# tachyon-beep/keisei

Hardware: AMD Instinct MI355X
Metric: PPO samples/sec, se_resnet 40x256 on 50x9x9 (higher is better)
Workload: dtype bf16; 1 GPU; se_resnet 40x256 KataGo-PPO minibatch step (gather+fwd+loss+bwd+clip+Adam), minibatch 4096/GPU from a 16384-sample device-resident epoch dataset, obs 50x9x9; per_gpu_batch=4096, global_batch=4096, parallelism=dp1

## Files before the change

include/keisei_amd.h:

```cpp
#ifndef KEISEI_AMD_H
#define KEISEI_AMD_H

#ifdef __cplusplus
extern "C" {
#endif

#define KA_OK 0
#define KA_ERR_ARG (-1)
#define KA_ERR_HIP (-2)
#define KA_ERR_UNSUPPORTED (-3)
#define KA_DTYPE_F32 0
#define KA_DTYPE_BF16 1

int ka_version(void);
const char* ka_target_arch(void);
const char* ka_last_error(void);
int ka_options_reload(void);

int ka_conv3x3_fwd(const void* in, const void* wpack, void* out, const float* in_scale, const float* in_shift,
                   const float* in_bias, int relu, float* bsum, float* sqpart, int B, int Cin, int Cout, int dtype,
                   void* stream);
int ka_conv3x3_fwd_keep_supported(int B, int Cin, int Cout, int dtype);
int ka_conv3x3_fwd_keep(const void* in, const void* wpack, void* out, const float* in_scale, const float* in_shift,
                        const float* in_bias, int relu, float* bsum, float* sqpart, void* x_out, int B, int Cin, int Cout, int dtype,
                        void* stream);
int ka_conv3x3_sqpart_rows(int B);
int ka_conv_route_counts(long long* out, int n);
int ka_conv3x3_dgrad_fused(const void* in, const void* in2, const float* k, void* dy_out, const void* wpack, void* out,
                           float* bsum, const void* ep_y, const float* ep_scale, const float* ep_shift,
                           const float* ep_mean, const float* ep_invstd, float* ep_s1, float* ep_s2, int B, int Cin,
                           int Cout, int dtype, void* stream);
int ka_conv3x3_dgrad_gated_supported(int B, int Cin, int Cout, int dtype, int masked);
int ka_conv3x3_dgrad_fused_gated(const void* du, const float* gate_add, const void* in2, const float* k,
                                 void* dy_out, const void* wpack, void* out, float* bsum, const void* ep_y,
                                 const float* ep_scale, const float* ep_shift, const float* ep_mean, const float* ep_invstd,
                                 float* ep_s1, float* ep_s2, int B, int Cin, int Cout, int dtype, void* stream);
int ka_pack_conv3x3(const float* w, void* dst, int Co, int Ci, int Nout, int Kin, int mode, int dtype, void* stream);
int ka_pack_conv3x3_multi(const long long* table, int n, long long max_pieces, int dtype, void* stream);
int ka_conv3x3_wgrad(const void* dy, const void* x, const float* in_scale, const float* in_shift, const float* in_bias,
                     int relu, float* slab, float* dw, int B, int Cin, int Cin_real, int Cout, int accumulate,
                     int target_wgs, int dtype, void* stream);
int ka_wgrad_splits(int B, int Cin, int Cout, int target_wgs);
int ka_debug_conv_stamps(unsigned long long* stamps);

int ka_obs_to_nhwc(const float* obs, const long long* idx, void* out, int B, int Cobs, int Cpad, int dtype, void* stream);
int ka_nhwc_to_nchw(const void* in, float* out, int B, int C, int dtype, void* stream);

int ka_reduce_workspace_doubles(int C);
int ka_bn_reduce(const float* bsum, int B, const float* sqpart, int R, int C, double* sums, double* part, void* stream);
int ka_bn_coeffs(const double* sums, double count, const double* count_dev, const float* gamma, const float* beta,
                 float* running_mean, float* running_var, long long* num_batches_tracked, float momentum, float eps,
                 float* scale, float* shift, float* mean, float* invstd, int C, void* stream);
int ka_bn_eval_coeffs(const float* gamma, const float* beta, const float* running_mean, const float* running_var,
                      float eps, float* scale, float* shift, int C, void* stream);
int ka_bn_eval_coeffs_multi(const long long* table, int n, int max_c, void* stream);
int ka_pair_reduce(const float* p1, const float* p2, int B, int C, double* sums, double* part, void* stream);
int ka_bn_bwd_coeffs(const double* sums_local, const double* sums_global, double count, const double* count_dev,
                     const float* gamma, const float* mean, const float* invstd, float* dgamma, float* dbeta, float* k,
                     int C, int train, void* stream);
int ka_sync_reduce(const float* p1, int rows1, const float* p2, int rows2, int C, double count, double* sums,
                   double* local_copy, double* part, void* stream);
int ka_bn_coeffs_parts(const double* part, double count, const float* gamma, const float* beta, float* running_mean,
                       float* running_var, long long* num_batches_tracked, float momentum, float eps, float* scale,
                       float* shift, float* mean, float* invstd, int C, void* stream);
int ka_bn_bwd_coeffs_parts(const double* part, double count, const float* gamma, const float* mean, const float* invstd,
                           float* dgamma, float* dbeta, float* k, int C, int train, void* stream);
int ka_bn_reduce_coeffs(const float* bsum, int B, const float* sqpart, int R, int C, double* part, int* counters, double count,
                        const float* gamma, const float* beta, float* running_mean, float* running_var,
                        long long* num_batches_tracked, float momentum, float eps, float* scale, float* shift, float* mean,
                        float* invstd, void* stream);
int ka_pair_reduce_bwd_coeffs(const float* p1, const float* p2, int rows, int C, double* part, int* counters, double count,
                              const float* gamma, const float* mean, const float* invstd, float* dgamma, float* dbeta, float* k,
                              int train, void* stream);
int ka_bn_bwd_apply(const void* dz, const void* y, const float* k, void* dy, int B, int C, int dtype, void* stream);
int ka_affine_rows(const float* in, const float* a, const float* s, float mul, float* out, int B, int C, void* stream);
// ... 287 lines not shown
```

keisei_amd/_lib.py:

```python
from __future__ import annotations

import ctypes
import os
from pathlib import Path
from typing import Optional

import torch

_LIB_PATH = Path(os.environ.get("KEISEI_AMD_LIB") or Path(__file__).resolve().parent / "libkeisei_amd.so")

_SIGS = {
    "ka_conv3x3_fwd": "pppppp i pp iii i p",
    "ka_conv3x3_fwd_keep_supported": "iiii",
    "ka_conv3x3_fwd_keep": "pppppp i pp p iii i p",
    "ka_conv3x3_dgrad_fused": "ppppp pp ppppp pp iii i p",
    "ka_conv3x3_dgrad_gated_supported": "iiiii",
    "ka_conv3x3_dgrad_fused_gated": "pppppp pp ppppp pp iii i p",
    "ka_conv3x3_sqpart_rows": "i",
    "ka_conv_route_counts": "p i",
    "ka_debug_conv_stamps": "p",
    "ka_pack_conv3x3": "pp iiii i i p",
    "ka_pack_conv3x3_multi": "p i q i p",
    "ka_wgrad_splits": "iiii",
    "ka_conv3x3_wgrad": "ppppp i pp iiii i i i p",
    "ka_obs_to_nhwc": "ppp iii i p",
    "ka_nhwc_to_nchw": "pp ii i p",
    "ka_bn_reduce": "p i p i i pp p",
    "ka_reduce_workspace_doubles": "i",
    "ka_pair_reduce": "pp ii pp p",
    "ka_sync_reduce": "p i p i i d ppp p",
    "ka_bn_coeffs": "p d p pppp p ff pppp i p",
    "ka_bn_coeffs_parts": "p d pppp p ff pppp i p",
    "ka_bn_bwd_coeffs_parts": "p d ppp ppp i i p",
    "ka_bn_reduce_coeffs": "p i p i i pp d pppp p ff pppp p",
    "ka_pair_reduce_bwd_coeffs": "pp i i pp d ppp ppp i p",
    "ka_bn_eval_coeffs": "pppp f pp i p",
    "ka_bn_bwd_coeffs": "pp d p ppp ppp i i p",
    "ka_affine_rows": "ppp f p ii p",
    "ka_bn_bwd_apply": "pppp ii i p",
    "ka_block_tail_fwd": "ppppp pp ii i p",
    "ka_block_tail_fwd_se_supported": "iii",
    "ka_block_tail_fwd_se": "pppppppp ppp ppp iii i p",
    "ka_pool_fwd": "pp ii i p",
    "ka_tail_bwd_reduce": "pppppp p ii i p",
    "ka_tail_bwd_dz": "ppppppp ppp ii i p",
    "ka_tail_bwd_fused_supported": "iii",
    "ka_tail_bwd_fused": "ppppp pppppp p pppp iii i p",
    "ka_relu_bn_bwd_reduce": "pppppp ppp ii i p",
    "ka_block_dx": "pppppp p ii i p",
    "ka_block_dx_tail_bwd_supported": "iii",
    "ka_block_dx_tail_bwd": "pppppp p ppppppppp p pppp iii i p",
    "ka_block_dx_tail_bwd_du": "ppppp p ppppppppp p pppp iii i p",
    "ka_block_dx_tail_bwd_du_gate": "ppppp p ppppppppp pp pppp iii i p",
    "ka_gemm": "pppp iii iii ii iii i i i p",
    "ka_reduce_slabs": "pp i q i p",
    "ka_reduce_slabs2": "pp q pp q i p",
    "ka_colsum": "pppp ii i p",
# ... 267 lines not shown
```

keisei_amd/csrc/wgrad.hip:

```cpp
#include <stdlib.h>
#include <type_traits>
#include "common.h"

namespace {

constexpr int kTC = 64;

struct WgradArgs {
    const void* dy;
    const void* x;
    const float* in_scale;
    const float* in_shift;
    const float* in_bias;
    float* slab;
    int B, Cin, Cout, relu, boards_per_split, ntn, ntiles, nsplit;
    int stagger;
    unsigned long long* stamps;
};

typedef __attribute__((address_space(3))) bf16x4* lds_bf16x4_ptr;

template <typename T, int TN> struct WG;
template <int TN> struct WG<bf16_t, TN> {
    static constexpr int KROWS = TN == 128 ? 82 : 96;
    static constexpr int PW = TN == 128 ? 17 : 11;
    static constexpr int SY = TN * 2 + 32;
    static constexpr int SX = kTC * 2 + 32;
};
template <int TN> struct WG<float, TN> {
    static constexpr int PW = 11;
    static constexpr int KROWS = 84;
    static constexpr int SY = TN * 4 + 64;
    static constexpr int SX = kTC * 4 + 64;
};

template <typename T, int TN, bool FUSED>
__global__ __launch_bounds__(TN * 4, TN == 64 ? 2 : 1) void wgrad_kernel(WgradArgs a) {
    typedef Elem<T> E;
    typedef typename E::vec16 vec16;
    constexpr int NTHR = TN * 4;
    constexpr int ESZ = E::kSize, P16 = E::kPer16;
    constexpr int SY = WG<T, TN>::SY, SX = WG<T, TN>::SX, KROWS = WG<T, TN>::KROWS;
    constexpr int PW = WG<T, TN>::PW, XSQ = 11 * PW;
    auto xsq = [](int p) { return (p / 9 + 1) * PW + (p % 9) + 1; };
    constexpr int PY = TN * ESZ / 16, PX = kTC * ESZ / 16;
    constexpr int NY = (KA_BOARD * PY + NTHR - 1) / NTHR, NX = (KA_BOARD * PX + NTHR - 1) / NTHR;
    extern __shared__ __attribute__((aligned(16))) char smem[];
    constexpr bool FLAT = sizeof(T) == 2 && TN == 128;
    constexpr int NBUF = FLAT ? 3 : ((sizeof(T) == 2) ? 2 : 1);
    constexpr int TILE_BYTES = KROWS * SY + XSQ * SX;
// ... 206 lines not shown
            }
        }
        }
        if (NBUF >= 2) {
            if (late) stage_next(b, ys, xs);
            __syncthreads();
        }
    };
    if (NSETS == 2) {
        for (int b = bbeg; b < bend; b += 2) {
            board_iter(b, ry[NSETS - 1], rx[NSETS - 1]);
            if (b + 1 < bend) board_iter(b + 1, ry[0], rx[0]);
        }
    } else {
#pragma unroll 1
        for (int b = bbeg; b < bend; ++b) board_iter(b, ry[0], rx[0]);
    }

    if (c_ok) {
        const int c = c0 + cq * 16 + r;
#pragma unroll
        for (int tap = 0; tap < 9; ++tap)
#pragma unroll
            for (int t = 0; t < 4; ++t)
#pragma unroll
                for (int i = 0; i < 4; ++i) {
                    const int n = n0 + (nh * 4 + t) * 16 + q * 4 + i;
                    if (n < a.Cout && c < a.Cin)
                        a.slab[(((size_t)split * 9 + tap) * a.Cout + n) * a.Cin + c] = acc[tap][t][i];
                }
    }
}

template <bool FUSED>
__global__ __launch_bounds__(512, 1) void wgrad_flat_kernel(WgradArgs a) {
    constexpr int NTHR = 512, SY = 128 * 2 + 32, SX = kTC * 2 + 32, KROWS = 82, PW = 17, XSQ = 11 * PW;
    constexpr int YB = KROWS * SY, TILE = YB + XSQ * SX, XTAB = 3 * TILE;
    constexpr int kTapBias = (PW + 1) * SX;
    constexpr bool PIPE = false;
    extern __shared__ __attribute__((aligned(16))) char smem[];
    const int tid = threadIdx.x, lane = tid & 63, wave = __builtin_amdgcn_readfirstlane(tid >> 6);
    const int r = lane & 15, q = lane >> 4;
    const int nh = wave & 1, cq = wave >> 1;
    const int xcd = blockIdx.x & 7, slot = blockIdx.x >> 3;
    const int tile = slot % a.ntiles;
    const int split = xcd + 8 * (slot / a.ntiles);
    if (split >= a.nsplit) return;
    const int tn = tile % a.ntn, tc = tile / a.ntn;
    const int n0 = tn * 128, c0 = tc * kTC;
    const int bbeg = split * a.boards_per_split;
    const int bend = min(a.B, bbeg + a.boards_per_split), nb = bend - bbeg;

    f32x4 acc[9][4];
#pragma unroll
    for (int t = 0; t < 9; ++t)
#pragma unroll
        for (int j = 0; j < 4; ++j) acc[t][j] = f32x4{0.f, 0.f, 0.f, 0.f};
    for (int i = tid; i < 3 * TILE / 16; i += NTHR) reinterpret_cast<uint4*>(smem)[i] = uint4{0, 0, 0, 0};
    if (tid < KROWS) {
        const int p = tid < KA_BOARD ? tid : 0;
        reinterpret_cast<int*>(smem + XTAB)[tid] = YB + ((p / 9 + 1) * PW + (p % 9) + 1) * SX;
    }

    const int yj = tid & 15, xj = tid & 7;
    const bool ycol_ok = n0 + yj * 8 < a.Cout, xcol_ok = c0 + xj * 8 < a.Cin;
    const __amdgpu_buffer_rsrc_t rs_y = __builtin_amdgcn_make_buffer_rsrc(const_cast<void*>(a.dy), 0, (unsigned)a.B * (KA_BOARD * 2u) * (unsigned)a.Cout, 0x00020000);
    const __amdgpu_buffer_rsrc_t rs_x = __builtin_amdgcn_make_buffer_rsrc(const_cast<void*>(a.x), 0, (unsigned)a.B * (KA_BOARD * 2u) * (unsigned)a.Cin, 0x00020000);
    const __amdgpu_buffer_rsrc_t rs_b = __builtin_amdgcn_make_buffer_rsrc(const_cast<float*>(FUSED ? a.in_bias : nullptr), 0,
                                                                          FUSED && a.in_bias ? (unsigned)a.B * 4u * (unsigned)a.Cin : 0u, 0x00020000);
    constexpr int kPark = 0x7fffffff;
    int ldsY[3], gY[3], ldsX[2], gX[2];
#pragma unroll
    for (int i = 0; i < 3; ++i) {
        const int row = (tid >> 4) + 32 * i;
        gY[i] = row < KA_BOARD && ycol_ok ? (row * a.Cout + n0 + yj * 8) * 2 : kPark;
        ldsY[i] = row < KA_BOARD ? row * SY + yj * 16 : 256;
    }
#pragma unroll
    for (int i = 0; i < 2; ++i) {
        const int row = (tid >> 3) + 64 * i;
        gX[i] = row < KA_BOARD && xcol_ok ? (row * a.Cin + c0 + xj * 8) * 2 : kPark;
        ldsX[i] = row < KA_BOARD ? YB + ((row / 9 + 1) * PW + (row % 9) + 1) * SX + xj * 16 : YB + (PW + 1) * SX + kTC * 2;
    }
    const int gB = xcol_ok ? (c0 + xj * 8) * 4 : kPark;
// ... 73 lines not shown
                tf = pad ? s_toff : tf;
            }
            yo[h] = tf + p * SY + coly;
            xo[h] = tf + *reinterpret_cast<const int*>(smem + XTAB + p * 4) + colx - kTapBias;
        }
        s_k += 32; s_p += 32;
        if (s_p >= KA_BOARD) { s_p -= KA_BOARD; s_toff = toff_next; }
    };

    if (a.stamps && tid == 0) {
        a.stamps[blockIdx.x * 8 + 0] = __builtin_amdgcn_s_memtime();
        a.stamps[blockIdx.x * 8 + 3] = __builtin_amdgcn_s_memrealtime();
    }
    if (nb > 0) load_board(bbeg);
    KA_LDS_BARRIER();
    if (nb > 0) {
        store_board(0);
        if (nb > 1) load_board(bbeg + 1);
    }
    prepare();
    KA_LDS_BARRIER();
    int ks = 0;
#ifdef KA_DIAG_WGRAD_TL
#define KA_TL(ph) do { if (a.stamps && blockIdx.x == 0 && jl >= 8 && jl < 24 && lane == 0) \
        a.stamps[4096 * 8 + ((jl - 8) * 8 + wave) * 8 + (ph)] = __builtin_amdgcn_s_memtime(); } while (0)
#else
#define KA_TL(ph) do {} while (0)
#endif
#pragma unroll 1
    for (int jl = 0; jl < nb; ++jl) {
        KA_TL(0);
        const int nxt = ((jl + 1) % 3) * TILE;
        auto stage_next = [&]() {
            if (jl + 1 < nb) {
                store_board(nxt);
                if (jl + 2 < nb) load_board(bbeg + jl + 2);
            }
        };
        if (!late) stage_next();
        KA_TL(1);
        const int ks_hi = jl + 1 == nb ? (KA_BOARD * nb + 31) / 32 : (KA_BOARD * (jl + 1)) / 32;
        if (!skip) {
            auto load_a = [&](bf16x8 (&f)[4]) {
#pragma unroll
                for (int t = 0; t < 4; ++t) {
                    bf16x4 lo = __builtin_amdgcn_ds_read_tr16_b64_v4bf16((lds_bf16x4_ptr)(smem + yo[0] + t * 32));
                    bf16x4 hi = __builtin_amdgcn_ds_read_tr16_b64_v4bf16((lds_bf16x4_ptr)(smem + yo[1] + t * 32));
                    f[t] = __builtin_shufflevector(lo, hi, 0, 1, 2, 3, 4, 5, 6, 7);
                }
            };
            auto kstep = [&](bf16x8 (&ac)[4], bf16x8 (&an)[4], bool more) {
                const int x0 = xo[0], x1 = xo[1];
                auto load_b = [&](int tap) {
                    const int toff = ((tap / 3 - 1) * PW + (tap % 3 - 1)) * SX + kTapBias;
                    bf16x4 lo = __builtin_amdgcn_ds_read_tr16_b64_v4bf16((lds_bf16x4_ptr)(smem + x0 + toff));
                    bf16x4 hi = __builtin_amdgcn_ds_read_tr16_b64_v4bf16((lds_bf16x4_ptr)(smem + x1 + toff));
                    return (bf16x8)__builtin_shufflevector(lo, hi, 0, 1, 2, 3, 4, 5, 6, 7);
                };
                bf16x8 bcur = load_b(0), bnx = load_b(1);
                prepare();
                if (PIPE && more) load_a(an);
#pragma unroll
                for (int tap = 0; tap < 9; ++tap) {
                    bf16x8 bn2 = bnx;
                    if (tap < 7) bn2 = load_b(tap + 2);
#pragma unroll
                    for (int t = 0; t < 4; ++t)
                        acc[tap][t] = __builtin_amdgcn_mfma_f32_16x16x32_bf16(ac[t], bcur, acc[tap][t], 0, 0, 0);
                    bcur = bnx; bnx = bn2;
// ... 26 lines not shown
        KA_TL(4);
    }
#undef KA_TL

    if (a.stamps && tid == 0) {
        a.stamps[blockIdx.x * 8 + 7] = __builtin_amdgcn_s_memtime();
        a.stamps[blockIdx.x * 8 + 4] = __builtin_amdgcn_s_memrealtime();
    }
    if (!skip) {
        const int c = c0 + cq * 16 + r;
        float* sl = a.slab + (size_t)split * 9 * a.Cout * a.Cin;
        const bool whole = n0 + nh * 64 + 64 <= a.Cout && c0 + cq * 16 + 16 <= a.Cin;
        if (whole) {
            float* base = sl + (size_t)(n0 + nh * 64 + q * 4) * a.Cin + c;
#pragma unroll
            for (int tap = 0; tap < 9; ++tap)
#pragma unroll
                for (int t = 0; t < 4; ++t)
#pragma unroll
                    for (int i = 0; i < 4; ++i)
                        base[((size_t)tap * a.Cout + t * 16 + i) * a.Cin] = acc[tap][t][i];
        } else {
#pragma unroll
            for (int tap = 0; tap < 9; ++tap)
#pragma unroll
                for (int t = 0; t < 4; ++t)
#pragma unroll
                    for (int i = 0; i < 4; ++i) {
                        const int n = n0 + (nh * 4 + t) * 16 + q * 4 + i;
                        if (n < a.Cout && c < a.Cin) sl[((size_t)tap * a.Cout + n) * a.Cin + c] = acc[tap][t][i];
                    }
        }
    }
}

__global__ void wgrad_reduce_kernel(const float* __restrict__ slab, float* __restrict__ dw, int nsplit, int Cout,
                                    int Cin, int Cin_real, int accumulate) {
    const int c4n = Cin >> 2;
    const size_t total = (size_t)9 * Cout * c4n, sstride = (size_t)9 * Cout * c4n;
    const f32x4* __restrict__ s4 = reinterpret_cast<const f32x4*>(slab);
    for (size_t i = blockIdx.x * (size_t)blockDim.x + threadIdx.x; i < total; i += (size_t)gridDim.x * blockDim.x) {
        const int c4 = (int)(i % c4n);
        const size_t tn = i / c4n;
        const int n = (int)(tn % Cout), tap = (int)(tn / Cout);
        f32x4 acc = {0.f, 0.f, 0.f, 0.f};
#pragma unroll 8
        for (int k = 0; k < nsplit; ++k) acc += s4[i + k * sstride];
#pragma unroll
        for (int e = 0; e < 4; ++e) {
            const int c = c4 * 4 + e;
            if (c < Cin_real) {
                const size_t o = ((size_t)n * Cin_real + c) * 9 + tap;
                dw[o] = accumulate ? dw[o] + acc[e] : acc[e];
            }
        }
    }
}

}

static int wgrad_tn(bool fused_input) {
    (void)fused_input;
    if (ka_opt(KA_OPT_WGRAD_TN, 128) == 64) return 64;
    return 128;
}

static int wgrad_splits_for(int B, int Cin, int Cout, int target_wgs) {
    const int tc = kTC;
    const int tn = 128;
    const int tiles = ((Cout + tn - 1) / tn) * ((Cin + tc - 1) / tc);
    if (const int v = ka_opt(KA_OPT_WGRAD_WGS, 0); v > 0) target_wgs = v;
    int s = (target_wgs > 0 ? target_wgs : 256) / tiles;
    if (s < 1) s = 1;
    if (s > B) s = B;
    const int bps = (B + s - 1) / s;
    return (B + bps - 1) / bps;
}

extern "C" int ka_wgrad_splits(int B, int Cin, int Cout, int target_wgs) { return wgrad_splits_for(B, Cin, Cout, target_wgs); }

template <bool FUSED>
static int launch_wgrad_flat(const WgradArgs& a, dim3 grid, hipStream_t st) {
    const size_t lds = 3 * (82 * (128 * 2 + 32) + 11 * 17 * (kTC * 2 + 32)) + 82 * 4;
    static std::atomic<unsigned long long> attr_done{0};
    if (int rc = ka_big_lds_once(reinterpret_cast<const void*>(&wgrad_flat_kernel<FUSED>), attr_done, "wgrad (lean)")) return rc;
    hipLaunchKernelGGL((wgrad_flat_kernel<FUSED>), grid, dim3(512), lds, st, a);
    return ka_check_launch("wgrad (lean)");
}

template <typename T, int TN, bool FUSED>
static int launch_wgrad(const WgradArgs& a, dim3 grid, hipStream_t st) {
    constexpr int NBUF = (sizeof(T) == 2 && TN == 128) ? 3 : (sizeof(T) == 2 ? 2 : 1);
    const size_t lds = (size_t)NBUF * (WG<T, TN>::KROWS * WG<T, TN>::SY + 11 * WG<T, TN>::PW * WG<T, TN>::SX);
    static std::atomic<unsigned long long> attr_done{0};
    if (int rc = ka_big_lds_once(reinterpret_cast<const void*>(&wgrad_kernel<T, TN, FUSED>), attr_done, "wgrad")) return rc;
    hipLaunchKernelGGL((wgrad_kernel<T, TN, FUSED>), grid, dim3(TN * 4), lds, st, a);
    return ka_check_launch("wgrad");
}

extern "C" int ka_conv3x3_wgrad(const void* dy, const void* x, const float* in_scale, const float* in_shift,
                                const float* in_bias, int relu, float* slab, float* dw, int B, int Cin, int Cin_real,
                                int Cout, int accumulate, int target_wgs, int dtype, void* stream) {
    KA_REQUIRE(dy && x && slab && dw && B > 0, "wgrad: null tensor");
    KA_REQUIRE(Cin % 16 == 0 && Cout % 16 == 0 && Cin_real <= Cin, "wgrad: need Cin,Cout %% 16 == 0");
    KA_REQUIRE((in_scale == nullptr) == (in_shift == nullptr), "wgrad: scale/shift must come together");
    hipStream_t st = static_cast<hipStream_t>(stream);
    const int tn = wgrad_tn(in_scale || in_bias || relu);
    const int nsplit = wgrad_splits_for(B, Cin, Cout, target_wgs);
    const int bps = (B + nsplit - 1) / nsplit;
    const int ntn = (Cout + tn - 1) / tn, ntiles = ntn * ((Cin + kTC - 1) / kTC);
    WgradArgs a{dy, x, in_scale, in_shift, in_bias, slab, B, Cin, Cout, relu, bps, ntn, ntiles, nsplit, ka_opt(KA_OPT_WGRAD_STAG, 1), ka_debug_stamps().load()};
    dim3 grid(8 * ntiles * ((nsplit + 7) / 8));
    int rc;
    const bool fused = in_scale || in_bias || relu;
#define KA_WG(T_, TN_) (fused ? launch_wgrad<T_, TN_, true>(a, grid, st) : launch_wgrad<T_, TN_, false>(a, grid, st))
    const bool fits32 = (unsigned long long)B * KA_BOARD * 2 * (unsigned long long)(Cin > Cout ? Cin : Cout) < 0x7fffffffull;
    const bool lean = dtype == KA_DTYPE_BF16 && tn == 128 && fits32 && ka_opt(KA_OPT_WGRAD_LEAN, 1) != 0;
    ka_conv_route(lean ? KA_RT_WGRAD_LEAN : KA_RT_WGRAD_TILED);
    if (lean)
        rc = fused ? launch_wgrad_flat<true>(a, grid, st) : launch_wgrad_flat<false>(a, grid, st);
    else if (dtype == KA_DTYPE_BF16) rc = tn == 64 ? KA_WG(bf16_t, 64) : KA_WG(bf16_t, 128);
    else if (dtype == KA_DTYPE_F32) rc = tn == 64 ? KA_WG(float, 64) : KA_WG(float, 128);
#undef KA_WG
    else { ka_set_error("wgrad: unknown dtype %d", dtype); return KA_ERR_ARG; }
    if (rc) return rc;
    const size_t total = (size_t)9 * Cout * (Cin / 4);
    const int blocks = (int)((total + 255) / 256 < 2048 ? (total + 255) / 256 : 2048);
    hipLaunchKernelGGL(wgrad_reduce_kernel, dim3(blocks), dim3(256), 0, st, slab, dw, nsplit, Cout, Cin, Cin_real,
                       accumulate);
    return ka_check_launch("wgrad_reduce");
}
```

keisei_amd/hip/seresnet.py:

```python
from __future__ import annotations

from typing import Dict, List, Optional

import gc
import os
import threading

import torch
import torch.distributed as dist
from torch import nn

from keisei_amd import _lib

_call = _lib.call


def _round_up(x: int, m: int) -> int:
    return (x + m - 1) // m * m


class _Saved:
    __slots__ = ("B", "T", "train", "xin", "stem", "blocks", "heads", "sync")


# ... 36 lines not shown
        if ev is None:
            _call(name, *args)
            return
        stream = torch.cuda.current_stream()
        a, b = torch.cuda.Event(enable_timing=True), torch.cuda.Event(enable_timing=True)
        a.record(stream)
        _call(name, *args)
        b.record(stream)
        ev[kind].append((a, b))
        if kind == "conv3x3" and name == "ka_conv3x3_fwd" and "conv3x3_fwd" in ev and self._in_forward:
            ev["conv3x3_fwd"].append((a, b))

    def notify_weights_updated(self) -> None:
        self.weights_epoch += 1

    def _red_ws(self, C: int, device) -> torch.Tensor:
        n = _lib.query("ka_reduce_workspace_doubles", C)
        if self._redws is None or self._redws.numel() < n or self._redws.device != device:
            self._redws = torch.empty(n, dtype=torch.float64, device=device)
        return self._redws

    def _red_counters(self, device) -> torch.Tensor:
        if self._redcnt is None or self._redcnt.device != device:
            self._redcnt = torch.zeros(64, dtype=torch.int32, device=device)
        return self._redcnt

    def _wgrad_side(self, n: int, device):
        if self._side is None or self._side.device != device:
            self._side = torch.cuda.Stream(device)
        if self._wslab is None or self._wslab.numel() < n or self._wslab.device != device:
            self._wslab = torch.empty(n, dtype=torch.float32, device=device)
        return self._side, self._wslab

    def _wgrad_launch(self, side, main, inputs, *args) -> None:
        if side is None:
            self._timed("wgrad", "ka_conv3x3_wgrad", *args, _lib.stream_ptr(main.device))
            return
        ev = torch.cuda.Event()
        ev.record(main)
        with torch.cuda.stream(side):
            side.wait_event(ev)
            self._timed("wgrad", "ka_conv3x3_wgrad", *args, _lib.stream_ptr(main.device))
        for t in inputs:
            t.record_stream(side)

    def _scratch_f32(self, n: int, device) -> torch.Tensor:
        if self._scratch is None or self._scratch.numel() < n or self._scratch.device != device:
            self._scratch = torch.empty(max(n, 1 << 20), dtype=torch.float32, device=device)
        return self._scratch

    def _conv_layers(self):
        m = self.model
        yield "input_conv", m.input_conv
        for i, blk in enumerate(m.blocks):
            yield f"blocks.{i}.conv1", blk.conv1
            yield f"blocks.{i}.conv2", blk.conv2

    def _get_packs(self, T: torch.dtype, device) -> Dict[str, tuple]:
        convs = list(self._conv_layers())
        tkey = (T, str(device), tuple(c.weight.data_ptr() for _, c in convs))
        ent = self._pack_sets.get(tkey)
        if ent is None:
            if len(self._pack_sets) >= 4:
                self._pack_sets.clear()
                self._graphs.clear()
            cpk = 32 if T == torch.bfloat16 else 16
            packs, jobs, mx = {}, [], 0
            for name, conv in convs:
                w = conv.weight
                co, ci = w.shape[0], w.shape[1]
                ci_pad = _round_up(ci, 64) if name == "input_conv" else ci
                nf = 9 * (ci_pad // cpk) * (co // 16) * 64
                fwd = torch.empty(nf * 16, dtype=torch.uint8, device=device)
                jobs.append([w.data_ptr(), fwd.data_ptr(), co, ci, co, ci_pad, 0, 0]); mx = max(mx, nf)
                dg = None
# ... 567 lines not shown
            grads["policy_conv2.weight"] = grads["policy_conv2.weight"].view_as(m.policy_conv2.weight)
            _call("ka_rows_bn_bwd", dp, p1, scp, shp, M, P, 0, st)
            nsp = max(1, min(256, (M + 2047) // 2048))
            part = torch.empty(nsp, P, device=dev); part2 = torch.empty(nsp, P, device=dev)
            mu_p, is_p = (mup, isp) if train else eval_stats(m.policy_bn1)
            _call("ka_rows_bn_sums", dp, p1, mu_p, is_p, part, part2, M, P, nsp, st)
            k = self._bn_backward(m.policy_bn1, part, part2, nsp, P, M, mu_p, is_p, train, grads, "policy_bn1", dev, st)
            _call("ka_rows_bn_bwd", dp, p1, k, None, M, P, 1, st)
            w1 = _FakeLinear(m.policy_conv1.weight.view(P, C), None)
            dxc = new_act()
            self._linear_bwd_act(dp, x, w1, grads, "policy_conv1.weight", dxc, bf, st)
            grads["policy_conv1.weight"] = grads["policy_conv1.weight"].view_as(m.policy_conv1.weight)
        else:
            for n, t in (("policy_conv2.weight", m.policy_conv2.weight), ("policy_conv2.bias", m.policy_conv2.bias),
                         ("policy_bn1.weight", m.policy_bn1.weight), ("policy_bn1.bias", m.policy_bn1.bias),
                         ("policy_conv1.weight", m.policy_conv1.weight)):
                grads[n] = torch.zeros_like(t)
        Hse = m.blocks[0].se_fc1.weight.shape[0] if len(m.blocks) > 0 else 0
        fuse_dx = (len(m.blocks) > 0 and os.environ.get("KA_DX_TAIL", "1") != "0"
                   and bool(_lib.query("ka_block_dx_tail_bwd_supported", C, Hse, code)))
        gate_dz = (fuse_dx and T == torch.bfloat16 and os.environ.get("KA_TAIL_GATE", "1") != "0"
                   and bool(_lib.query("ka_conv3x3_dgrad_gated_supported", B, C, C, code, 1)))
        pend = (dxc, None, None, x, pool, dpool, new_act())
        dout = pend[6]
        if not fuse_dx:
            _call("ka_block_dx", *pend, B, C, code, st)
            pend = None

        s1p = torch.empty(B, C, device=dev); s2p = torch.empty(B, C, device=dev)
        twg = 192 if self.overlap_wgrad else 0
        nsplit = _lib.query("ka_wgrad_splits", B, C, C, twg)
        nslab = max(nsplit * 9 * C * C, _lib.query("ka_wgrad_splits", B, 64, C, 0) * 9 * C * 64)
        main = torch.cuda.current_stream(dev)
        side, slab = self._wgrad_side(nslab, dev)
        if not self.overlap_wgrad:
            side = None

        red = self.grad_reducer
        per_block = 2 * 9 * C * C
        blocks_per_bucket = max(1, red.bucket_bytes // (4 * per_block)) if red is not None else 0
        bucket, bucket_off, bucket_left = None, 0, 0

        def conv_grad(like, i, last):
            nonlocal bucket, bucket_off, bucket_left
            if red is None:
                return torch.empty_like(like)
            if bucket is None:
                bucket_left = min(blocks_per_bucket, i + 1)
                bucket = torch.empty(bucket_left * per_block, device=dev)
                bucket_off = 0
            n = like.numel()
            view = bucket[bucket_off:bucket_off + n].view_as(like)
            bucket_off += n
            return view

        def conv_grads_done(i):
            nonlocal bucket, bucket_left
            if red is None:
                return
            bucket_left -= 1
            if bucket_left == 0:
                ev = torch.cuda.Event()
                ev.record(side if side is not None else main)
                red.launch(bucket, f"conv[{i}:{i + bucket.numel() // per_block}]", ev)
                bucket = None

        fc_bwd_side = None
        if os.environ.get("KA_FC_BWD_SIDE", "0") == "1" and fc_tr is not None and not self.overlap_wgrad:
            if self._fc_side is None or self._fc_side.device != dev:
                self._fc_side = torch.cuda.Stream(dev)
            fc_bwd_side = self._fc_side
        self._gpool_done = None

        def gpool_join():
            if self._gpool_done is not None:
                main.wait_event(self._gpool_done)
                self._gpool_done = None

        for i in range(len(sv.blocks) - 1, -1, -1):
            blk = m.blocks[i]
            (bx, bpool, y1, sc1, sh1, mu1, is1, g1, g, y2, sc2, sh2, mu2, is2, sqz, se1, se, out, x2) = sv.blocks[i]
            pre = f"blocks.{i}."
            if not train:
                mu1, is1 = eval_stats(blk.bn1); mu2, is2 = eval_stats(blk.bn2)
            dse = torch.empty(B, 2 * C, device=dev)
            H = blk.se_fc1.weight.shape[0]
            gpool_join()
            gate_add = None
            if pend is not None and gate_dz:
                dse1 = torch.empty(B, H, device=dev)
                gate_add = torch.empty(2, B, C, device=dev)
                dz = pend[6]
                _call("ka_block_dx_tail_bwd_du_gate", pend[0], pend[1], *pend[3:], y2, sc2, sh2, se, se1, blk.se_fc2.weight,
                      blk.se_fc1.weight, mu2, is2, gate_add[0], gate_add[1], dse, dse1, s1p, s2p, B, C, H, code, st)
                self._linear_bwd(dse, se1, blk.se_fc2, grads, pre + "se_fc2.weight", pre + "se_fc2.bias", st, need_dx=False)
                self._linear_bwd(dse1, sqz, blk.se_fc1, grads, pre + "se_fc1.weight", pre + "se_fc1.bias", st, need_dx=False)
            elif pend is not None:
                dse1 = torch.empty(B, H, device=dev)
                dz = new_act()
                _call("ka_block_dx_tail_bwd_du", pend[0], pend[1], *pend[3:], y2, sc2, sh2, se, se1, blk.se_fc2.weight,
                      blk.se_fc1.weight, mu2, is2, dz, dse, dse1, s1p, s2p, B, C, H, code, st)
                self._linear_bwd(dse, se1, blk.se_fc2, grads, pre + "se_fc2.weight", pre + "se_fc2.bias", st, need_dx=False)
                self._linear_bwd(dse1, sqz, blk.se_fc1, grads, pre + "se_fc1.weight", pre + "se_fc1.bias", st, need_dx=False)
            elif _lib.query("ka_tail_bwd_fused_supported", C, H, code):
                dse1 = torch.empty(B, H, device=dev)
                dz = new_act()
                _call("ka_tail_bwd_fused", dout, out, y2, sc2, sh2, se, se1, blk.se_fc2.weight, blk.se_fc1.weight, mu2, is2,
                      dz, dse, dse1, s1p, s2p, B, C, H, code, st)
                self._linear_bwd(dse, se1, blk.se_fc2, grads, pre + "se_fc2.weight", pre + "se_fc2.bias", st, need_dx=False)
                self._linear_bwd(dse1, sqz, blk.se_fc1, grads, pre + "se_fc1.weight", pre + "se_fc1.bias", st, need_dx=False)
            else:
                dz = new_act()
                _call("ka_tail_bwd_reduce", dout, out, y2, sc2, sh2, se, dse, B, C, code, st)
                dse1 = self._linear_bwd(dse, se1, blk.se_fc2, grads, pre + "se_fc2.weight", pre + "se_fc2.bias", st)
                _call("ka_relu_mask", dse1, se1, dse1.numel(), st)
                dsq = self._linear_bwd(dse1, sqz, blk.se_fc1, grads, pre + "se_fc1.weight", pre + "se_fc1.bias", st)
                _call("ka_tail_bwd_dz", dout, out, y2, se, dsq, mu2, is2, dz, s1p, s2p, B, C, code, st)
            k2 = self._bn_backward(blk.bn2, s1p, s2p, B, C, count, mu2, is2, train, grads, pre + "bn2", dev, st)
            dg = torch.empty(B, C, device=dev)
            if T == torch.bfloat16:
                rows = _lib.query("ka_conv3x3_sqpart_rows", B)
                dy2, dh = new_act(), new_act()
                ep1 = torch.empty(rows, C, device=dev); ep2 = torch.empty(rows, C, device=dev)
                if gate_add is not None:
                    self._timed("conv3x3", "ka_conv3x3_dgrad_fused_gated", dz, gate_add, y2, k2, dy2, packs[pre + "conv2"][1], dh, dg,
                                y1, sc1, sh1, mu1, is1, ep1, ep2, B, C, C, code, st)
                else:
                    self._timed("conv3x3", "ka_conv3x3_dgrad_fused", dz, y2, k2, dy2, packs[pre + "conv2"][1], dh, dg,
                                y1, sc1, sh1, mu1, is1, ep1, ep2, B, C, C, code, st)
                dW2 = conv_grad(blk.conv2.weight, i, False)
                if x2 is not None:
                    self._wgrad_launch(side, main, (dy2, dW2), dy2, x2, None, None, None, 0, slab, dW2, B, C, C, C, 0, twg, code)
                else:
                    self._wgrad_launch(side, main, (dy2, dW2), dy2, y1, sc1, sh1, g, 1, slab, dW2, B, C, C, C, 0, twg, code)
                grads[pre + "conv2.weight"] = dW2
                gside = None
                if fc_bwd_side is not None:
                    gev = torch.cuda.Event(); gev.record(main)
                    gside = (fc_bwd_side, gev)
                bn1_ctx = self._bn_backward_begin(blk.bn1, ep1, ep2, rows, C, count, train, dev, st)
                dpool_x = self._gpool_bwd(i, blk, dg, g1, bpool, grads, pre, st, fc_tr, gside)
                k1 = self._bn_backward_end(bn1_ctx, blk.bn1, C, count, mu1, is1, train, grads, pre + "bn1", dev, st)
                dy1, dxc = new_act(), new_act()
                self._timed("conv3x3", "ka_conv3x3_dgrad_fused", dh, y1, k1, dy1, packs[pre + "conv1"][1], dxc, None,
                            None, None, None, None, None, None, None, B, C, C, code, st)
                dW1 = conv_grad(blk.conv1.weight, i, True)
                self._wgrad_launch(side, main, (dy1, dW1), dy1, bx, None, None, None, 0, slab, dW1, B, C, C, C, 0, twg, code)
                grads[pre + "conv1.weight"] = dW1
                conv_grads_done(i)
                dx = new_act()
            else:
                _call("ka_bn_bwd_apply", dz, y2, k2, dz, B, C, code, st)
                dh = new_act()
                self._timed("conv3x3", "ka_conv3x3_fwd", dz, packs[pre + "conv2"][1], dh, None, None, None, 0, dg, None, B, C, C, code, st)
                dW2 = conv_grad(blk.conv2.weight, i, False)
                self._wgrad_launch(side, main, (dz, dW2), dz, y1, sc1, sh1, g, 1, slab, dW2, B, C, C, C, 0, twg, code)
                grads[pre + "conv2.weight"] = dW2
                dpool_x = self._gpool_bwd(i, blk, dg, g1, bpool, grads, pre, st, fc_tr)
                _call("ka_relu_bn_bwd_reduce", dh, y1, sc1, sh1, mu1, is1, dh, s1p, s2p, B, C, code, st)
                k1 = self._bn_backward(blk.bn1, s1p, s2p, B, C, count, mu1, is1, train, grads, pre + "bn1", dev, st)
                _call("ka_bn_bwd_apply", dh, y1, k1, dh, B, C, code, st)
                dxc = new_act() if side is not None else dz
                self._timed("conv3x3", "ka_conv3x3_fwd", dh, packs[pre + "conv1"][1], dxc, None, None, None, 0, None, None, B, C, C, code, st)
                dW1 = conv_grad(blk.conv1.weight, i, True)
                self._wgrad_launch(side, main, (dh, dW1), dh, bx, None, None, None, 0, slab, dW1, B, C, C, C, 0, twg, code)
                grads[pre + "conv1.weight"] = dW1
                conv_grads_done(i)
                dx = new_act() if side is not None else dh
            if fuse_dx and i > 0:
                pend = (dxc, dout, out, bx, bpool, dpool_x, dx)
            else:
                gpool_join()
                _call("ka_block_dx", dxc, dout, out, bx, bpool, dpool_x, dx, B, C, code, st)
                pend = None
            dout = dx

        y0, sc0, sh0, mu0, is0 = sv.stem
        if not train:
            mu0, is0 = eval_stats(m.input_bn)
        _call("ka_relu_bn_bwd_reduce", dout, y0, sc0, sh0, mu0, is0, dout, s1p, s2p, B, C, code, st)
        k0 = self._bn_backward(m.input_bn, s1p, s2p, B, C, count, mu0, is0, train, grads, "input_bn", dev, st)
        _call("ka_bn_bwd_apply", dout, y0, k0, dout, B, C, code, st)
        dW0 = torch.empty_like(m.input_conv.weight)
        cin_pad = sv.xin.shape[2]
        self._wgrad_launch(side, main, (dout, dW0), dout, sv.xin, None, None, None, 0, slab, dW0, B, cin_pad,
                           p.obs_channels, C, 0, 0, code)
        grads["input_conv.weight"] = dW0
        fc_flat = self._flush_fc_jobs(grads, dev, st)
        if side is not None:
            main.wait_stream(side)
        if red is not None:
            in_flat = set()
            if fc_flat is not None:
                lo, hi = fc_flat.data_ptr(), fc_flat.data_ptr() + 4 * fc_flat.numel()
                in_flat = {n for n, t in grads.items() if lo <= t.data_ptr() < hi}
                red.launch(fc_flat, "fc", red._event_now(fc_flat))
            small_names = [n for n, t in grads.items()
                           if n not in in_flat and not (n.startswith("blocks.") and n.endswith(("conv1.weight", "conv2.weight")))]
            for n in small_names:
                red.add_small(grads[n])
            for n, v in zip(small_names, red.finish()):
                grads[n] = v
        return grads

    def _linear_bwd_act(self, dy, x_act, lin, grads, wname, dx_act, bf, st):
        M, N = dy.shape
        K = lin.weight.shape[1]
        dev = dy.device
        ns = max(1, min(_FC_SPLITS, (M + 1023) // 1024))
        dW = torch.empty(N, K, device=dev)
        slab = self._scratch_f32(ns * N * K, dev)
        self._gemm(dy, x_act, slab, None, N, K, M, N, K, K, 1, 0, st, bbf=bf, ns=ns)
        _call("ka_reduce_slabs", slab, dW, ns, N * K, 0, st)
        grads[wname] = dW
        self._gemm(dy, lin.weight, dx_act, None, M, K, N, N, K, K, 0, 0, st, cbf=bf)


class _FakeLinear:
    __slots__ = ("weight", "bias")
# ... 48 lines not shown
```

Baseline: 43160 samples/s.

## Defer wgrad split-K reductions into later wgrad kernels via rotating slabs

Adds a deferred wgrad path. Each conv weight-gradient kernel writes its per-split partial slab, and that slab is reduced into dW later, either inside a subsequent unfused wgrad launch (up to two pending jobs, paced across the board loop with buffer loads) or by an explicit flush kernel. Three rotating slab buffers replace the single one, and bucket bookkeeping is reworked so gradient-reducer launches fire only after the deferred reductions complete. The aim is to remove separate reduce kernel launches and hide the reduce memory traffic behind wgrad compute. In exchange it uses three times the slab memory and adds register pressure and extra loads inside the main wgrad kernel.

```diff
diff --git a/include/keisei_amd.h b/include/keisei_amd.h
--- a/include/keisei_amd.h
+++ b/include/keisei_amd.h
@@ -41,6 +41,16 @@
                      int relu, float* slab, float* dw, int B, int Cin, int Cin_real, int Cout, int accumulate,
                      int target_wgs, int dtype, void* stream);
 int ka_wgrad_splits(int B, int Cin, int Cout, int target_wgs);
+int ka_conv3x3_wgrad_deferred_supported(int B, int Cin, int Cout, int dtype);
+int ka_conv3x3_wgrad_carry_slots(int fused_input);
+int ka_conv3x3_wgrad_deferred(const void* dy, const void* x, const float* in_scale, const float* in_shift, const float* in_bias,
+                              int relu, float* slab, int B, int Cin, int Cout, int target_wgs, int dtype,
+                              const float* p0_slab, float* p0_dw, int p0_nsplit, int p0_Cout, int p0_Cin, int p0_Cin_real,
+                              int p0_accumulate,
+                              const float* p1_slab, float* p1_dw, int p1_nsplit, int p1_Cout, int p1_Cin, int p1_Cin_real,
+                              int p1_accumulate, void* stream);
+int ka_conv3x3_wgrad_flush(const float* slab, float* dw, int nsplit, int Cout, int Cin, int Cin_real, int accumulate,
+                           void* stream);
 int ka_debug_conv_stamps(unsigned long long* stamps);
 
 int ka_obs_to_nhwc(const float* obs, const long long* idx, void* out, int B, int Cobs, int Cpad, int dtype, void* stream);
diff --git a/keisei_amd/_lib.py b/keisei_amd/_lib.py
--- a/keisei_amd/_lib.py
+++ b/keisei_amd/_lib.py
@@ -23,6 +23,10 @@
     "ka_pack_conv3x3_multi": "p i q i p",
     "ka_wgrad_splits": "iiii",
     "ka_conv3x3_wgrad": "ppppp i pp iiii i i i p",
+    "ka_conv3x3_wgrad_deferred_supported": "iiii",
+    "ka_conv3x3_wgrad_carry_slots": "i",
+    "ka_conv3x3_wgrad_deferred": "ppppp i p iii i i pp iiiii pp iiiii p",
+    "ka_conv3x3_wgrad_flush": "pp iiiii p",
     "ka_obs_to_nhwc": "ppp iii i p",
     "ka_nhwc_to_nchw": "pp ii i p",
     "ka_bn_reduce": "p i p i i pp p",
diff --git a/keisei_amd/csrc/wgrad.hip b/keisei_amd/csrc/wgrad.hip
--- a/keisei_amd/csrc/wgrad.hip
+++ b/keisei_amd/csrc/wgrad.hip
@@ -5,6 +5,12 @@
 namespace {
 
 constexpr int kTC = 64;
+
+struct WgradJob {
+    const float* slab;
+    float* dw;
+    int nsplit, Cout, Cin, Cin_real, accumulate;
+};
 
 struct WgradArgs {
     const void* dy;
@@ -16,6 +22,9 @@
     int B, Cin, Cout, relu, boards_per_split, ntn, ntiles, nsplit;
     int stagger;
     unsigned long long* stamps;
+    WgradJob job[2];
+    int njobs;
+    int pace;
 };
 
 typedef __attribute__((address_space(3))) bf16x4* lds_bf16x4_ptr;
@@ -288,7 +297,7 @@
     }
 }
 
-template <bool FUSED>
+template <bool FUSED, int NP = 0>
 __global__ __launch_bounds__(512, 1) void wgrad_flat_kernel(WgradArgs a) {
     constexpr int NTHR = 512, SY = 128 * 2 + 32, SX = kTC * 2 + 32, KROWS = 82, PW = 17, XSQ = 11 * PW;
     constexpr int YB = KROWS * SY, TILE = YB + XSQ * SX, XTAB = 3 * TILE;
@@ -301,11 +310,74 @@
     const int xcd = blockIdx.x & 7, slot = blockIdx.x >> 3;
     const int tile = slot % a.ntiles;
     const int split = xcd + 8 * (slot / a.ntiles);
-    if (split >= a.nsplit) return;
+
+    const unsigned pg = blockIdx.x * 512u + tid, pG = gridDim.x * 512u, pgw = blockIdx.x * 512u + wave * 64u;
+    int pj = 0, pk = 0, pn = 0, pvoff = 0;
+    unsigned pbase = 0;
+    f32x4 pacc = {0.f, 0.f, 0.f, 0.f}, pp[NP > 0 ? NP : 1];
+#define KA_PJ(f) (pj == 0 ? a.job[0].f : a.job[1].f)
+    auto pend_consume = [&]() {
+        if constexpr (NP > 0) {
+            if (pn == 0) return;
+            const unsigned c4n = (unsigned)KA_PJ(Cin) >> 2, Cout = KA_PJ(Cout), total = 9u * Cout * c4n;
+            const bool live = pbase + pgw < total;
+            if (live) {
+#pragma unroll
+                for (int e = 0; e < NP; ++e)
+                    if (e < pn) pacc += pp[e];
+            }
+            pk += pn; pn = 0;
+            if (pk < KA_PJ(nsplit)) return;
+            const unsigned i = pbase + pg;
+            if (live && i < total) {
+                const unsigned c4 = i % c4n, tn_ = i / c4n, n = tn_ % Cout, tap = tn_ / Cout;
+                const int cr = KA_PJ(Cin_real), accum = KA_PJ(accumulate);
+                float* dw = KA_PJ(dw);
+#pragma unroll
+                for (int e = 0; e < 4; ++e) {
+                    const int c = (int)c4 * 4 + e;
+                    if (c < cr) {
+                        const size_t o = ((size_t)n * cr + c) * 9 + tap;
+                        dw[o] = accum ? dw[o] + pacc[e] : pacc[e];
+                    }
+                }
+            }
+            pk = 0; pbase += pG;
+            if (pbase >= total) { pbase = 0; ++pj; }
+        }
+    };
+    auto pend_issue = [&]() {
+        if constexpr (NP > 0) {
+            if (pj >= a.njobs) return;
+            const int ns = KA_PJ(nsplit);
+            const unsigned total = 9u * (unsigned)KA_PJ(Cout) * ((unsigned)KA_PJ(Cin) >> 2);
+            const int sstride = (int)(total * 16u);
+            pn = min(NP, ns - pk);
+            if (pbase + pgw >= total) return;
+            const __amdgpu_buffer_rsrc_t rs = __builtin_amdgcn_make_buffer_rsrc(const_cast<float*>(KA_PJ(slab)), 0, (unsigned)ns * (unsigned)sstride, 0x00020000);
+            if (pk == 0) {
+                const unsigned i = pbase + pg;
+                pvoff = i < total ? (int)(i * 16u) : 0x7fffffff;
+                pacc = f32x4{0.f, 0.f, 0.f, 0.f};
+            }
+            const int so = pk * sstride;
+#pragma unroll
+            for (int e = 0; e < NP; ++e)
+                if (e < pn) pp[e] = __builtin_bit_cast(f32x4, __builtin_amdgcn_raw_buffer_load_b128(rs, pvoff, so + e * sstride, 0));
+        }
+    };
+    auto pend_drain = [&]() {
+        if constexpr (NP > 0) {
+            while (pn != 0 || pj < a.njobs) { pend_consume(); pend_issue(); }
+        }
+    };
+
+    if (split >= a.nsplit) { pend_drain(); return; }
     const int tn = tile % a.ntn, tc = tile / a.ntn;
     const int n0 = tn * 128, c0 = tc * kTC;
     const int bbeg = split * a.boards_per_split;
     const int bend = min(a.B, bbeg + a.boards_per_split), nb = bend - bbeg;
+    int pwait = 0;
 
     f32x4 acc[9][4];
 #pragma unroll
@@ -445,9 +517,13 @@
         KA_TL(0);
         const int nxt = ((jl + 1) % 3) * TILE;
         auto stage_next = [&]() {
+            pend_consume();
             if (jl + 1 < nb) {
                 store_board(nxt);
                 if (jl + 2 < nb) load_board(bbeg + jl + 2);
+            }
+            if constexpr (NP > 0) {
+                if (pwait == 0) { pend_issue(); pwait = a.pace - 1; } else --pwait;
             }
         };
         if (!late) stage_next();
@@ -540,6 +616,8 @@
                     }
         }
     }
+    pend_drain();
+#undef KA_PJ
 }
 
 __global__ void wgrad_reduce_kernel(const float* __restrict__ slab, float* __restrict__ dw, int nsplit, int Cout,
@@ -587,12 +665,12 @@
 
 extern "C" int ka_wgrad_splits(int B, int Cin, int Cout, int target_wgs) { return wgrad_splits_for(B, Cin, Cout, target_wgs); }
 
-template <bool FUSED>
+template <bool FUSED, int NP = 0>
 static int launch_wgrad_flat(const WgradArgs& a, dim3 grid, hipStream_t st) {
     const size_t lds = 3 * (82 * (128 * 2 + 32) + 11 * 17 * (kTC * 2 + 32)) + 82 * 4;
     static std::atomic<unsigned long long> attr_done{0};
-    if (int rc = ka_big_lds_once(reinterpret_cast<const void*>(&wgrad_flat_kernel<FUSED>), attr_done, "wgrad (lean)")) return rc;
-    hipLaunchKernelGGL((wgrad_flat_kernel<FUSED>), grid, dim3(512), lds, st, a);
+    if (int rc = ka_big_lds_once(reinterpret_cast<const void*>(&wgrad_flat_kernel<FUSED, NP>), attr_done, "wgrad (lean)")) return rc;
+    hipLaunchKernelGGL((wgrad_flat_kernel<FUSED, NP>), grid, dim3(512), lds, st, a);
     return ka_check_launch("wgrad (lean)");
 }
 
@@ -638,3 +716,70 @@
                        accumulate);
     return ka_check_launch("wgrad_reduce");
 }
+
+constexpr int kCarryPiecesPlain = 4;
+constexpr int kCarrySlotsPlain = 2, kCarrySlotsFused = 0;
+
+static bool wgrad_lean_ok(int B, int Cin, int Cout, int dtype) {
+    const bool fits32 = (unsigned long long)B * KA_BOARD * 2 * (unsigned long long)(Cin > Cout ? Cin : Cout) < 0x7fffffffull;
+    return dtype == KA_DTYPE_BF16 && wgrad_tn(false) == 128 && fits32 && ka_opt(KA_OPT_WGRAD_LEAN, 1) != 0 && B > 0 &&
+           Cin > 0 && Cout > 0 && Cin % 16 == 0 && Cout % 16 == 0;
+}
+
+extern "C" int ka_conv3x3_wgrad_deferred_supported(int B, int Cin, int Cout, int dtype) { return wgrad_lean_ok(B, Cin, Cout, dtype) ? 1 : 0; }
+
+extern "C" int ka_conv3x3_wgrad_carry_slots(int fused_input) { return fused_input ? kCarrySlotsFused : kCarrySlotsPlain; }
+
+static int wgrad_job_check(const WgradJob& j) {
+    KA_REQUIRE(j.slab && j.dw && j.nsplit > 0 && j.Cout > 0 && j.Cin > 0, "wgrad: bad pending job");
+    KA_REQUIRE(j.Cin % 4 == 0 && j.Cin_real > 0 && j.Cin_real <= j.Cin, "wgrad: pending job needs Cin %% 4 == 0, Cin_real <= Cin");
+    return 0;
+}
+
+extern "C" int ka_conv3x3_wgrad_flush(const float* slab, float* dw, int nsplit, int Cout, int Cin, int Cin_real, int accumulate,
+                                      void* stream) {
+    const WgradJob j{slab, dw, nsplit, Cout, Cin, Cin_real, accumulate};
+    if (int rc = wgrad_job_check(j)) return rc;
+    const size_t total = (size_t)9 * Cout * (Cin / 4);
+    const int blocks = (int)((total + 255) / 256 < 2048 ? (total + 255) / 256 : 2048);
+    hipLaunchKernelGGL(wgrad_reduce_kernel, dim3(blocks), dim3(256), 0, static_cast<hipStream_t>(stream), slab, dw, nsplit, Cout,
+                       Cin, Cin_real, accumulate);
+    return ka_check_launch("wgrad_reduce");
+}
+
+extern "C" int ka_conv3x3_wgrad_deferred(const void* dy, const void* x, const float* in_scale, const float* in_shift,
+                                         const float* in_bias, int relu, float* slab, int B, int Cin, int Cout, int target_wgs,
+                                         int dtype,
+                                         const float* p0_slab, float* p0_dw, int p0_nsplit, int p0_Cout, int p0_Cin, int p0_Cin_real, int p0_accumulate,
+                                         const float* p1_slab, float* p1_dw, int p1_nsplit, int p1_Cout, int p1_Cin, int p1_Cin_real, int p1_accumulate,
+                                         void* stream) {
+    KA_REQUIRE(dy && x && slab && B > 0, "wgrad: null tensor");
+    KA_REQUIRE(Cin % 16 == 0 && Cout % 16 == 0, "wgrad: need Cin,Cout %% 16 == 0");
+    KA_REQUIRE((in_scale == nullptr) == (in_shift == nullptr), "wgrad: scale/shift must come together");
+    KA_REQUIRE(wgrad_lean_ok(B, Cin, Cout, dtype), "wgrad: deferred reduce needs the lean kernel (ka_conv3x3_wgrad_deferred_supported)");
+    KA_REQUIRE(p0_slab || !p1_slab, "wgrad: pending job 1 without job 0");
+    hipStream_t st = static_cast<hipStream_t>(stream);
+    const bool fused = in_scale || in_bias || relu;
+    const int nsplit = wgrad_splits_for(B, Cin, Cout, target_wgs);
+    const int bps = (B + nsplit - 1) / nsplit;
+    const int ntn = (Cout + 127) / 128, ntiles = ntn * ((Cin + kTC - 1) / kTC);
+    WgradArgs a{dy, x, in_scale, in_shift, in_bias, slab, B, Cin, Cout, relu, bps, ntn, ntiles, nsplit, ka_opt(KA_OPT_WGRAD_STAG, 1), ka_debug_stamps().load()};
+    if (p0_slab) a.job[a.njobs++] = WgradJob{p0_slab, p0_dw, p0_nsplit, p0_Cout, p0_Cin, p0_Cin_real, p0_accumulate};
+    if (p1_slab) a.job[a.njobs++] = WgradJob{p1_slab, p1_dw, p1_nsplit, p1_Cout, p1_Cin, p1_Cin_real, p1_accumulate};
+    KA_REQUIRE(a.njobs <= (fused ? kCarrySlotsFused : kCarrySlotsPlain), "wgrad: this input form carries fewer pending jobs (ka_conv3x3_wgrad_carry_slots)");
+    for (int j = 0; j < a.njobs; ++j) {
+        if (int rc = wgrad_job_check(a.job[j])) return rc;
+        KA_REQUIRE(a.job[j].slab != slab, "wgrad: a pending job's slabs are the launch's own slab buffer");
+        KA_REQUIRE((unsigned long long)a.job[j].nsplit * 9 * a.job[j].Cout * a.job[j].Cin * 4 < 0x7fffffffull, "wgrad: pending job's slabs exceed the 32-bit descriptor range: flush it");
+    }
+    dim3 grid(8 * ntiles * ((nsplit + 7) / 8));
+    long long groups = 2;
+    for (int j = 0; j < a.njobs; ++j) {
+        const long long total = 9ll * a.job[j].Cout * (a.job[j].Cin / 4), thr = 512ll * grid.x;
+        groups += (total + thr - 1) / thr * ((a.job[j].nsplit + kCarryPiecesPlain - 1) / kCarryPiecesPlain);
+    }
+    a.pace = (int)(bps / groups > 1 ? bps / groups : 1);
+    ka_conv_route(KA_RT_WGRAD_LEAN);
+    if (fused) return launch_wgrad_flat<true>(a, grid, st);
+    return launch_wgrad_flat<false, kCarryPiecesPlain>(a, grid, st);
+}
diff --git a/keisei_amd/hip/seresnet.py b/keisei_amd/hip/seresnet.py
--- a/keisei_amd/hip/seresnet.py
+++ b/keisei_amd/hip/seresnet.py
@@ -92,15 +92,15 @@
             self._wslab = torch.empty(n, dtype=torch.float32, device=device)
         return self._side, self._wslab
 
-    def _wgrad_launch(self, side, main, inputs, *args) -> None:
+    def _wgrad_launch(self, side, main, inputs, *args, name="ka_conv3x3_wgrad") -> None:
         if side is None:
-            self._timed("wgrad", "ka_conv3x3_wgrad", *args, _lib.stream_ptr(main.device))
+            self._timed("wgrad", name, *args, _lib.stream_ptr(main.device))
             return
         ev = torch.cuda.Event()
         ev.record(main)
         with torch.cuda.stream(side):
             side.wait_event(ev)
-            self._timed("wgrad", "ka_conv3x3_wgrad", *args, _lib.stream_ptr(main.device))
+            self._timed("wgrad", name, *args, _lib.stream_ptr(main.device))
         for t in inputs:
             t.record_stream(side)
 
@@ -734,38 +734,84 @@
         nsplit = _lib.query("ka_wgrad_splits", B, C, C, twg)
         nslab = max(nsplit * 9 * C * C, _lib.query("ka_wgrad_splits", B, 64, C, 0) * 9 * C * 64)
         main = torch.cuda.current_stream(dev)
-        side, slab = self._wgrad_side(nslab, dev)
+        cin_pad = sv.xin.shape[2]
+        defer = (os.environ.get("KA_WGRAD_DEFER", "1") != "0"
+                 and bool(_lib.query("ka_conv3x3_wgrad_deferred_supported", B, C, C, code))
+                 and bool(_lib.query("ka_conv3x3_wgrad_deferred_supported", B, cin_pad, C, code)))
+        nslab = (nslab + 3) // 4 * 4
+        side, slab = self._wgrad_side(3 * nslab if defer else nslab, dev)
+        wslabs = [slab[k * nslab:(k + 1) * nslab] for k in range(3)] if defer else None
+        wpend = []
         if not self.overlap_wgrad:
             side = None
 
         red = self.grad_reducer
         per_block = 2 * 9 * C * C
         blocks_per_bucket = max(1, red.bucket_bytes // (4 * per_block)) if red is not None else 0
-        bucket, bucket_off, bucket_left = None, 0, 0
+        bucket, bucket_off, fill_left = None, 0, 0
+        open_buckets = []
 
         def conv_grad(like, i, last):
-            nonlocal bucket, bucket_off, bucket_left
+            nonlocal bucket, bucket_off, fill_left
             if red is None:
                 return torch.empty_like(like)
             if bucket is None:
-                bucket_left = min(blocks_per_bucket, i + 1)
-                bucket = torch.empty(bucket_left * per_block, device=dev)
+                fill_left = min(blocks_per_bucket, i + 1)
+                bucket = torch.empty(fill_left * per_block, device=dev)
                 bucket_off = 0
+                open_buckets.append([bucket, fill_left])
             n = like.numel()
             view = bucket[bucket_off:bucket_off + n].view_as(like)
             bucket_off += n
+            if last:
+                fill_left -= 1
+                if fill_left == 0:
+                    bucket = None
             return view
 
         def conv_grads_done(i):
-            nonlocal bucket, bucket_left
             if red is None:
                 return
-            bucket_left -= 1
-            if bucket_left == 0:
+            ent = open_buckets[0]
+            ent[1] -= 1
+            if ent[1] == 0:
+                open_buckets.pop(0)
                 ev = torch.cuda.Event()
                 ev.record(side if side is not None else main)
-                red.launch(bucket, f"conv[{i}:{i + bucket.numel() // per_block}]", ev)
-                bucket = None
+                red.launch(ent[0], f"conv[{i}:{i + ent[0].numel() // per_block}]", ev)
+
+        def wgrad_flush_oldest():
+            bi, dW_, ns_, co_, ci_, cr_, done_ = wpend.pop(0)
+            if side is None:
+                _call("ka_conv3x3_wgrad_flush", wslabs[bi], dW_, ns_, co_, ci_, cr_, 0, _lib.stream_ptr(dev))
+            else:
+                with torch.cuda.stream(side):
+                    _call("ka_conv3x3_wgrad_flush", wslabs[bi], dW_, ns_, co_, ci_, cr_, 0, _lib.stream_ptr(dev))
+            if done_ is not None:
+                conv_grads_done(done_)
+
+        def wgrad(inputs, dy_, x_, sc_, sh_, bias_, relu_, dW_, cin, cin_real, twg_, done=None):
+            if not defer:
+                self._wgrad_launch(side, main, inputs, dy_, x_, sc_, sh_, bias_, relu_, slab, dW_, B, cin, cin_real, C, 0, twg_, code)
+                if done is not None:
+                    conv_grads_done(done)
+                return
+            fused = int(sc_ is not None or bias_ is not None or bool(relu_))
+            while len(wpend) >= len(wslabs):
+                wgrad_flush_oldest()
+            carried = wpend[:_lib.query("ka_conv3x3_wgrad_carry_slots", fused)]
+            del wpend[:len(carried)]
+            free = next(k for k in range(len(wslabs)) if all(e[0] != k for e in wpend + carried))
+            jobs = []
+            for k in range(2):
+                e = carried[k] if k < len(carried) else None
+                jobs += [wslabs[e[0]], e[1], e[2], e[3], e[4], e[5], 0] if e is not None else [None, None, 0, 0, 0, 0, 0]
+            self._wgrad_launch(side, main, inputs, dy_, x_, sc_, sh_, bias_, relu_, wslabs[free], B, cin, C, twg_, code, *jobs,
+                               name="ka_conv3x3_wgrad_deferred")
+            for e in carried:
+                if e[6] is not None:
+                    conv_grads_done(e[6])
+            wpend.append([free, dW_, _lib.query("ka_wgrad_splits", B, cin, C, twg_), C, cin, cin_real, done])
 
         fc_bwd_side = None
         if os.environ.get("KA_FC_BWD_SIDE", "0") == "1" and fc_tr is not None and not self.overlap_wgrad:
@@ -832,9 +878,9 @@
                                 y1, sc1, sh1, mu1, is1, ep1, ep2, B, C, C, code, st)
                 dW2 = conv_grad(blk.conv2.weight, i, False)
                 if x2 is not None:
-                    self._wgrad_launch(side, main, (dy2, dW2), dy2, x2, None, None, None, 0, slab, dW2, B, C, C, C, 0, twg, code)
+                    wgrad((dy2, dW2), dy2, x2, None, None, None, 0, dW2, C, C, twg)
                 else:
-                    self._wgrad_launch(side, main, (dy2, dW2), dy2, y1, sc1, sh1, g, 1, slab, dW2, B, C, C, C, 0, twg, code)
+                    wgrad((dy2, dW2), dy2, y1, sc1, sh1, g, 1, dW2, C, C, twg)
                 grads[pre + "conv2.weight"] = dW2
                 gside = None
                 if fc_bwd_side is not None:
@@ -847,16 +893,15 @@
                 self._timed("conv3x3", "ka_conv3x3_dgrad_fused", dh, y1, k1, dy1, packs[pre + "conv1"][1], dxc, None,
                             None, None, None, None, None, None, None, B, C, C, code, st)
                 dW1 = conv_grad(blk.conv1.weight, i, True)
-                self._wgrad_launch(side, main, (dy1, dW1), dy1, bx, None, None, None, 0, slab, dW1, B, C, C, C, 0, twg, code)
+                wgrad((dy1, dW1), dy1, bx, None, None, None, 0, dW1, C, C, twg, done=i)
                 grads[pre + "conv1.weight"] = dW1
-                conv_grads_done(i)
                 dx = new_act()
             else:
                 _call("ka_bn_bwd_apply", dz, y2, k2, dz, B, C, code, st)
                 dh = new_act()
                 self._timed("conv3x3", "ka_conv3x3_fwd", dz, packs[pre + "conv2"][1], dh, None, None, None, 0, dg, None, B, C, C, code, st)
                 dW2 = conv_grad(blk.conv2.weight, i, False)
-                self._wgrad_launch(side, main, (dz, dW2), dz, y1, sc1, sh1, g, 1, slab, dW2, B, C, C, C, 0, twg, code)
+                wgrad((dz, dW2), dz, y1, sc1, sh1, g, 1, dW2, C, C, twg)
                 grads[pre + "conv2.weight"] = dW2
                 dpool_x = self._gpool_bwd(i, blk, dg, g1, bpool, grads, pre, st, fc_tr)
                 _call("ka_relu_bn_bwd_reduce", dh, y1, sc1, sh1, mu1, is1, dh, s1p, s2p, B, C, code, st)
@@ -865,9 +910,8 @@
                 dxc = new_act() if side is not None else dz
                 self._timed("conv3x3", "ka_conv3x3_fwd", dh, packs[pre + "conv1"][1], dxc, None, None, None, 0, None, None, B, C, C, code, st)
                 dW1 = conv_grad(blk.conv1.weight, i, True)
-                self._wgrad_launch(side, main, (dh, dW1), dh, bx, None, None, None, 0, slab, dW1, B, C, C, C, 0, twg, code)
+                wgrad((dh, dW1), dh, bx, None, None, None, 0, dW1, C, C, twg, done=i)
                 grads[pre + "conv1.weight"] = dW1
-                conv_grads_done(i)
                 dx = new_act() if side is not None else dh
             if fuse_dx and i > 0:
                 pend = (dxc, dout, out, bx, bpool, dpool_x, dx)
@@ -884,9 +928,9 @@
         k0 = self._bn_backward(m.input_bn, s1p, s2p, B, C, count, mu0, is0, train, grads, "input_bn", dev, st)
         _call("ka_bn_bwd_apply", dout, y0, k0, dout, B, C, code, st)
         dW0 = torch.empty_like(m.input_conv.weight)
-        cin_pad = sv.xin.shape[2]
-        self._wgrad_launch(side, main, (dout, dW0), dout, sv.xin, None, None, None, 0, slab, dW0, B, cin_pad,
-                           p.obs_channels, C, 0, 0, code)
+        wgrad((dout, dW0), dout, sv.xin, None, None, None, 0, dW0, cin_pad, p.obs_channels, 0)
+        while wpend:
+            wgrad_flush_oldest()
         grads["input_conv.weight"] = dW0
         fc_flat = self._flush_fc_jobs(grads, dev, st)
         if side is not None:
```

Measured after the change: 43240 samples/s, median of 5. About the same (+0.2%).
